# yaoyongxin/dmft-ed

Hardware: AMD Instinct MI355X
Metric: Lanczos SpMV GB/s + ground-state iters/s, Ns=16 half-filled sector, 1/2/4/8 GPU (higher is better)
Workload: dtype f64; 1 GPU; c2: Norb=1 Nbath=7 (Nlevels=16) half-filled (4,4) sector, dim 4900, stored real(8) H, plain Lanczos 512 iters/step, persistent MODE 4 (4 = stored matrix in the Kronecker register layout); parallelism=sector replicas x1

## Files before the change

dmft-ed_amd/csrc/ed_host.hpp:

```cpp
#pragma once
#include <hip/hip_runtime.h>
#include <stdint.h>

#include <string>

#include "../../include/ed_gpu.h"

std::string& ed_err_slot();
static inline int fail(int code, const std::string& msg) {
  ed_err_slot() = msg;
  return code;
}
#define HIPCK(x)                                                                       \
  do {                                                                                 \
    hipError_t e_ = (x);                                                               \
    if (e_ != hipSuccess)                                                              \
      return fail(ED_ERR_HIP, std::string(#x) + " -> " + hipGetErrorString(e_));       \
  } while (0)
#define CK(x)                  \
  do {                         \
    int r_ = (x);              \
    if (r_ != ED_OK) return r_; \
  } while (0)

namespace edg {

constexpr bool pkr_fits(int E, int RPT) { return RPT * (3 * E + 8) + 3 * E <= 216; }
constexpr bool pkr_fits_c512(int E, int RPT) { return E == 4 ? RPT <= 10 : RPT <= 6; }
constexpr int preg_cap(bool hc, bool vc) { return vc ? (hc ? 80 : 84) : 112; }
static inline int persist_rpt01(int64_t dim) {
  const int64_t rpt = (dim + 1024 - 1) / 1024;
  return rpt <= 6 ? (int)rpt : rpt <= 8 ? 8 : rpt <= 10 ? 10 : rpt <= 12 ? 12 : 16;
}

struct PersistGeom {
  int64_t dim = 0;
  int preg_E = 0, preg_rpt = 0, kreg_W = 0, kreg_rpt = 0, pkr_E = 0, pkr_rpt = 0;
};

int persist_launch(bool hc, bool vc, int mode, const PersistGeom& g, const void* run, int64_t lds,
                   hipStream_t st, int nb);

}
```

dmft-ed_amd/csrc/ed_lib.hip:

```cpp
#include <hip/hip_runtime.h>
#include <math.h>
#include <stdint.h>
#include <stdio.h>
#include <string.h>

#include <algorithm>
#include <atomic>
#include <condition_variable>
#include <functional>
#include <mutex>
#include <thread>
#include <string>
#include <map>
#include <vector>

#include "ed_kernels.hpp"
#include "ed_persist.hpp"
#include "ed_trlan.hpp"
#include "ed_trlbatch.hpp"
#include "ed_trlmulti.hpp"
#include "ed_fused.hpp"
#include "ed_split.hpp"
#include "ed_tables.hpp"
#include "ed_host.hpp"
// ... 92 lines not shown
  int split_uch = 8;
  SplitSlice* d_bsl = nullptr;
  int nbsl = 0;
  int2* d_itR = nullptr;
  int* d_glist = nullptr;
  int* d_xoff = nullptr;
  int2* d_ul = nullptr;
  uint32_t* d_lw = nullptr;
  int64_t nul = 0, nlw = 0, nfar = 0, nfar_u = 0;
  bool fused = false;
  FuUnit* d_fu = nullptr;
  int64_t nfu = 0;
  uint32_t* d_fa = nullptr;
  int2* d_ful = nullptr;
  uint32_t* d_flw = nullptr;
  int64_t fu_na = 0, fu_nu = 0, fu_nl = 0, fu_far = 0, fu_far_u = 0;
  int fu_wa_max = 0, fu_wa_min = 0, fu_uch = kFuUChunk;
  DirChunk* d_dchunk = nullptr;
  int ndchunk = 0;
  DirChunk* d_dchunk2 = nullptr;
  int ndchunk2 = 0;
  DirGroup* d_dops = nullptr;
  uint16_t *d_rank16 = nullptr, *d_pat16 = nullptr;
  void* d_ddiag = nullptr;
  bool dir_patlds = false;
  int dir_lds = 0, dir_grid = 0;
  bool kron = false;
  KronHost K;
  void *d_x = nullptr, *d_y = nullptr;
  LancWS ws;
  int64_t bytes = 0;
  std::vector<void*> allocs;
  double pthresh = 0.0;
  int preg_E = 0;
  int preg_rpt = 0;
  int kreg_W = 0, kreg_rpt = 0;
  uint32_t* d_pk = nullptr;
  void* d_dict = nullptr;
  int ndict = 0;
  int pkr_state = 0;
  int pkr_src = -1;
  int pkr_E = 0, pkr_rpt = 0, pkr_du = 0, pkr_dd = 0, pkr_degu = 0, pkr_degd = 0;
  const int32_t *d_kupc = nullptr, *d_kdwc = nullptr;
  const double *d_kupv = nullptr, *d_kdwv = nullptr, *d_kdiag = nullptr;
  hipGraphExec_t gexec = nullptr;
  int g_path = -2, g_vc = -1, g_chunk = 0;
  bool g_basis = false;
};

static int dcopy(const ed_sector* s, void* dst, const void* src, size_t n, hipMemcpyKind k) {
  HIPCK(hipMemcpyAsync(dst, src, n, k, s->stream));
  HIPCK(hipStreamSynchronize(s->stream));
  return ED_OK;
}
static int dalloc(ed_sector* s, void** p, size_t n) {
  if (n == 0) n = 16;
  hipError_t e = hipMallocAsync(p, n, s->stream);
  if (e != hipSuccess) {
    *p = nullptr;
    return fail(e == hipErrorOutOfMemory ? ED_ERR_OOM : ED_ERR_HIP,
                std::string("hipMalloc(") + std::to_string(n) + ") -> " + hipGetErrorString(e));
  }
  s->allocs.push_back(*p);
  s->bytes += (int64_t)n;
  return ED_OK;
}
static void dfree(ed_sector* s, void** p, size_t n) {
  if (!*p) return;
  auto it = std::find(s->allocs.begin(), s->allocs.end(), *p);
  if (it != s->allocs.end()) s->allocs.erase(it);
  (void)hipFreeAsync(*p, s->stream);
  s->bytes -= (int64_t)n;
  *p = nullptr;
}
template <class T>
static int dalloc_t(ed_sector* s, T** p, size_t count) {
  return dalloc(s, (void**)p, count * sizeof(T));
}
template <class T>
static int upload(ed_sector* s, T** p, const std::vector<T>& h) {
  CK(dalloc_t(s, p, h.size()));
  return dcopy(s, *p, h.data(), h.size() * sizeof(T), hipMemcpyHostToDevice);
}

static std::mutex g_pin_mu;
static std::multimap<size_t, void*> g_pin_free;
static std::map<void*, size_t> g_pin_size;
static void* pinned_get(size_t n) {
  {
    std::lock_guard<std::mutex> lk(g_pin_mu);
    auto it = g_pin_free.lower_bound(n);
    if (it != g_pin_free.end()) {
      void* p = it->second;
      g_pin_free.erase(it);
      return p;
    }
  }
  n = std::max<size_t>(n, 4096);
  void* p = nullptr;
  if (hipHostMalloc(&p, n, hipHostMallocDefault) != hipSuccess) return nullptr;
  std::lock_guard<std::mutex> lk(g_pin_mu);
  g_pin_size[p] = n;
  return p;
}
static void pinned_put(void* p) {
  if (!p) return;
  std::lock_guard<std::mutex> lk(g_pin_mu);
  g_pin_free.emplace(g_pin_size[p], p);
}
struct PinnedLease {
  void* const p;
  const hipStream_t st;
  PinnedLease(size_t n, hipStream_t st_) : p(pinned_get(n)), st(st_) {}
  PinnedLease(const PinnedLease&) = delete;
  ~PinnedLease() {
    if (!p) return;
    (void)hipStreamSynchronize(st);
    pinned_put(p);
  }
};
struct DevFree {
  void* p;
  hipStream_t st;
  ~DevFree() { (void)hipFreeAsync(p, st); }
};
static inline size_t even(size_t q) { return (q + 1) & ~(size_t)1; }

static void sector_free(ed_sector* s) {
  if (!s) return;
  (void)hipSetDevice(s->device);
  if (s->gexec) (void)hipGraphExecDestroy(s->gexec);
  for (hipEvent_t& e : s->ws.ev)
    if (e) (void)hipEventDestroy(e);
// ... 1578 lines not shown
  const int64_t du = K.dimup;
  std::vector<int32_t> uc((size_t)K.degup * du);
  std::vector<double> uv((size_t)K.degup * du);
  if (K.degup) {
    CK(dcopy(s, uc.data(), K.upc, uc.size() * 4, hipMemcpyDeviceToHost));
    CK(dcopy(s, uv.data(), K.upv, uv.size() * 8, hipMemcpyDeviceToHost));
  }
  std::vector<std::vector<PkrHop>> ul(du);
  for (int64_t r = 0; r < du; r++)
    for (int e = 0; e < K.degup; e++) {
      uint64_t bits;
      memcpy(&bits, &uv[(size_t)e * du + r], 8);
      ul[r].push_back({uc[(size_t)e * du + r], bits});
    }
  pkr_order_up(ul, (int)du, s->pkr_E);
  s->pkr_degu = s->pkr_E;
  CK(pkr_upload(s, ul, s->pkr_degu, du, &s->d_kupc, &s->d_kupv));
  s->d_kdwc = K.dwc;
  s->d_kdwv = (const double*)K.dwv;
  s->d_kdiag = nullptr;
  s->pkr_state = 1;
  return 1;
}

static int64_t persist_lds(const ed_sector* s, int vc, int mode);
static int64_t persist_vrows(const ed_sector* s, int mode, int vc = 0) {
  switch (mode) {
    case 2: return (int64_t)kPRegBlock * s->preg_rpt;
    case 3: return (int64_t)kPRegBlock * s->kreg_rpt;
    case 4: return (int64_t)kPRegBlock * s->pkr_rpt;
    default: return (int64_t)kPBlock * persist_rpt01(s->dim);
  }
}
static int persist_mode(ed_sector* s, int vc, int path) {
  const int o = s->opts;
  if (o & ED_OPT_NO_PERSIST) return -1;
  const int64_t vs = vc ? 16 : 8;
  const int64_t rpt_max = (vc || s->hc) ? 5 : 8;
  if (s->dim > rpt_max * (int64_t)kPBlock) return -1;
  int64_t lds = ((persist_vrows(s, 0) * vs + 15) & ~(int64_t)15);
  if (!(o & (ED_OPT_NO_PKRON | ED_OPT_NO_PREG)) &&
      ((path == 0 && !(o & ED_OPT_PERSIST_STORED) && build_pkron_stored(s) > 0) ||
       (path == 2 && build_pkron_direct(s) > 0)) &&
      (vc == 0 || pkr_fits_c512(s->pkr_E, s->pkr_rpt)) &&
      persist_lds(s, vc, 4) <= kLdsBudget)
    return 4;
  if (path == 0) {
    if (o & ED_OPT_PERSIST_STORED) return lds <= kLdsBudget ? 0 : -1;
    if (o & ED_OPT_NO_PREG) return -1;
    if (s->dim > 10 * (int64_t)kPRegBlock) return -1;
    const int W = build_preg(s);
    if (W < 0) return -1;
    if (s->preg_rpt * W > preg_cap(s->hc, vc)) return -1;
    if (persist_lds(s, vc, 2) > kLdsBudget) return -1;
    return 2;
  }
  if (path == 2 && !(o & ED_OPT_NO_PREG) && s->dim <= 10 * (int64_t)kPRegBlock) {
    const KronHost& K = s->K;
    const int deg = K.degup + K.degdw;
    int W = 0;
    for (int w : {8, 12, 14, 16})
      if (!W && deg <= w) W = w;
    const int64_t rpt = (s->dim + kPRegBlock - 1) / kPRegBlock;
    const int RPT = rpt <= 2 ? 2 : rpt <= 4 ? 4 : rpt <= 6 ? 6 : rpt <= 8 ? 8 : 10;
    const int64_t hs = s->hc ? 16 : 8;
    const int64_t dict = ((int64_t)(K.degup * K.dimup + K.degdw * K.dimdw) + 1) * hs;
    const int cap = preg_cap(s->hc, vc);
// ... 12 lines not shown
           (int64_t)K.nimp * K.nimp * 8 + 256;
    return lds <= kLdsBudget ? 1 : -1;
  }
  return -1;
}

static int64_t persist_lds(const ed_sector* s, int vc, int mode) {
  const int64_t vs = vc ? 16 : 8, vr = persist_vrows(s, mode, vc);
  int64_t lds = ((vr * vs + 15) & ~(int64_t)15);
  if (mode == 4) {
    if (!vc) return (((vr + vr / kPRegBlock) * vs + 15) & ~(int64_t)15);
    return lds + (int64_t)s->pkr_E * s->pkr_dd * 8;
  }
  if (mode == 2) {
    const int64_t hs = s->hc ? 16 : 8;
    return lds + ((vr * 8 + 15) & ~(int64_t)15) + (((int64_t)s->ndict * hs + 15) & ~(int64_t)15);
  }
  if (mode == 3) {
    const int64_t hs = s->hc ? 16 : 8;
    const int64_t dict = ((int64_t)(s->K.degup * s->K.dimup + s->K.degdw * s->K.dimdw) + 1) * hs;
    return lds + ((vr * 8 + 15) & ~(int64_t)15) + ((dict + 15) & ~(int64_t)15);
  }
  if (mode == 1) {
    const KronHost& K = s->K;
    const int64_t hs = s->hc ? 16 : 8;
    auto al = [](int64_t b) { return (b + 15) & ~(int64_t)15; };
    lds += al(K.dimup * hs) + al(K.dimdw * hs) + al((int64_t)K.degup * K.dimup * hs) +
           al((int64_t)K.degdw * K.dimdw * hs) + al((int64_t)K.degup * K.dimup * 4) +
           al((int64_t)K.degdw * K.dimdw * 4) + al(K.dimup) + al(K.dimdw) + al((int64_t)K.nimp * K.nimp * 8);
  }
  return lds;
}

static PersistGeom persist_geom(const ed_sector* s) {
  PersistGeom g;
  g.dim = s->dim;
  g.preg_E = s->preg_E;
  g.preg_rpt = s->preg_rpt;
  g.kreg_W = s->kreg_W;
  g.kreg_rpt = s->kreg_rpt;
  g.pkr_E = s->pkr_E;
  g.pkr_rpt = s->pkr_rpt;
  return g;
}

struct PersistBatch {
  int nb;
  void *R, *P;
  LancState* st;
  double *alpha, *beta;
  int64_t ldr, ldp, ldab;
};

template <bool VC>
static int persist_iters(ed_sector* s, int mode, bool basis, int niter, int first, hipStream_t st,
                         const PersistBatch* bt = nullptr) {
  LancWS& w = s->ws;
  const int nb = bt ? bt->nb : 1;
  auto fill = [&](auto& r) {
    using RT = std::remove_reference_t<decltype(r)>;
    using HT = std::remove_const_t<std::remove_pointer_t<decltype(r.diag)>>;
    memset(&r, 0, sizeof(RT));
    r.diag = (const HT*)s->d_diag;
    r.sptr = s->d_sptr;
    r.cols = s->d_cols;
    r.vals = (const HT*)s->d_vals;
    r.dim = s->dim;
    r.R = w.R;
    r.P = w.P;
    r.st = w.st;
    r.alpha = w.alpha;
    r.beta = w.beta;
    r.basis = basis ? w.basis : nullptr;
    r.niter = niter;
    r.first = first;
    r.thresh = s->pthresh;
    r.pk = s->d_pk;
    r.dict = (const HT*)s->d_dict;
    r.ndict = s->ndict;
    r.kupc = s->d_kupc;
    r.kupv = s->d_kupv;
    r.kdwc = s->d_kdwc;
    r.kdwv = s->d_kdwv;
    r.kdiag = s->d_kdiag;
    r.kdu = s->pkr_du;
    r.kdd = s->pkr_dd;
    r.kdegu = s->pkr_degu;
    r.kdegd = s->pkr_degd;
    if (bt) {
      r.R = bt->R;
      r.P = bt->P;
      r.st = bt->st;
      r.alpha = bt->alpha;
      r.beta = bt->beta;
      r.basis = nullptr;
      r.ldr = bt->ldr;
      r.ldp = bt->ldp;
      r.ldab = bt->ldab;
    }
  };
  const int64_t lds = persist_lds(s, VC, mode);
  if (s->hc) {
    if constexpr (!VC) return fail(ED_ERR_ARG, "complex H needs complex vectors");
    else {
      PersistRun<true> r;
      fill(r);
      if (mode == 1 || mode == 3) r.K = kron_args<true>(s);
      if (mode == 4) return fail(ED_ERR_UNSUPPORTED, "MODE 4 needs real H");
      return persist_launch(true, true, mode, persist_geom(s), &r, lds, st, nb);
    }
  }
  PersistRun<false> r;
  fill(r);
  if (mode == 1 || mode == 3 || (mode == 4 && s->kron)) r.K = kron_args<false>(s);
  return persist_launch(false, VC, mode, persist_geom(s), &r, lds, st, nb);
}

static int persist_set_thresh(ed_sector* s, double thresh, hipStream_t st) {
  s->pthresh = thresh;
  HIPCK(hipMemsetAsync(s->ws.st, 0, sizeof(LancState), st));
  HIPCK(hipMemsetAsync(s->ws.alpha, 0, 2 * (s->ws.cap + 2) * sizeof(double), st));
  return ED_OK;
}


__global__ void k_hash_vec(double* v, int64_t n, uint64_t seed) {
  for (int64_t i = (int64_t)blockIdx.x * kBlock + threadIdx.x; i < n; i += (int64_t)gridDim.x * kBlock) {
    v[i] = hash_vec_unit(i, seed);
  }
}

template <bool VC>
struct Trlan {
  using V = val_t<VC>;
  ed_sector* s = nullptr;
  int path = 0;
  hipStream_t st = nullptr;
  int64_t dim = 0;
  int G = 1, m = 0, mcap = 0;
  bool fused = true;
  V *Vb = nullptr, *Xb = nullptr, *w = nullptr;
  double2 *h = nullptr, *coef = nullptr, *part = nullptr, *part2 = nullptr;
  int kFinFoldG = 256;
  bool graphs_on = true;
  bool solo = true;
  bool locupd = true;
  int* lof = nullptr;
  double *Y = nullptr, *npart = nullptr, *alpha = nullptr, *beta = nullptr;
  double *npA = nullptr, *npB = nullptr;
  double* hp = nullptr;
  std::vector<void*> mine;
  std::vector<std::pair<int, hipGraphExec_t>> graphs;
  int nhv = 0;
  ~Trlan() {
// ... 1040 lines not shown
  if (hipStreamSynchronize(s->stream) != hipSuccess) {
    sector_free(s);
    return fail(ED_ERR_HIP, "sector build");
  }
#undef TRY
  *out = s;
  return ED_OK;
}

int ed_sector_create(const ed_params* p, int32_t q1, int32_t q2, int32_t flags, int32_t device,
                     void* stream, ed_sector** out) {
  return sector_create(p, q1, q2, flags, 0, -1, device, (hipStream_t)stream, out);
}

int ed_sector_create_rows(const ed_params* p, int32_t q1, int32_t q2, int32_t flags, int64_t row0,
                          int64_t nrows, int32_t device, void* stream, ed_sector** out) {
  return sector_create(p, q1, q2, flags, row0, nrows, device, (hipStream_t)stream, out);
}

int ed_sector_destroy(ed_sector* s) {
  sector_free(s);
  return ED_OK;
}

static constexpr int32_t kOptKnown =
    ED_OPT_NO_PERSIST | ED_OPT_PERSIST_STORED | ED_OPT_NO_PREG | ED_OPT_NO_PKRON | ED_OPT_SPLIT_SIMPLE |
    ED_OPT_NO_BATCH | ED_OPT_EIGH_NO_VERIFY | ED_OPT_TRLAN_UNFUSED | ED_OPT_TRLAN_NOFOLD | ED_OPT_NO_GRAPH |
    ED_OPT_TRLAN_NOLOCAL | ED_OPT_TRLAN_NOSOLO | ED_OPT_TRLAN_FULLUPD | ED_OPT_STORED_EXACT |
    ED_OPT_EIGH_FULLPROBE | ED_OPT_NO_FUSED | ED_OPT_EIGH_NOHINT;

int ed_sector_set_options(ed_sector* s, int32_t opts) {
  if (!s) return fail(ED_ERR_ARG, "null");
  if (opts & ~kOptKnown) return fail(ED_ERR_ARG, "unknown ED_OPT_* bits");
  if (opts != s->opts) drop_graph(s);
  s->opts = opts;
  return ED_OK;
}

int ed_sector_get_info(const ed_sector* s, ed_sector_info* info) {
  if (!s || !info) return fail(ED_ERR_ARG, "null");
  memset(info, 0, sizeof(*info));
  info->dim = s->dim;
  info->row0 = s->row0;
  info->nrows = s->nrows;
  info->nnz = (s->flags & ED_STORED) ? s->nnz : 0;
  info->padded = s->padded;
  info->ns = s->Mh.ns;
  info->mode = s->Mh.mode;
  info->q1 = s->T.q1;
  info->q2 = s->T.q2;
  info->flags = s->flags;
  info->kron = s->kron ? 1 : 0;
  info->dimup = s->T.dimup;
  info->dimdw = s->T.dimdw;
  info->device_bytes = s->bytes;
  info->packed = s->d_words ? 1 : 0;
  info->npdict = s->npdict;
  info->split = s->split ? 1 : 0;
  info->split_far = s->nfar;
  info->split_far_uniform = s->nfar_u;
  info->fused = s->fused ? 1 : 0;
  info->fused_far = s->fu_far;
  info->fused_far_uniform = s->fu_far_u;
  info->fused_bytes = s->fused ? (s->fu_na + s->fu_nl) * 4 + s->fu_nu * 8 + s->nfu * (int64_t)sizeof(FuUnit) : 0;
  info->split_bytes = s->split ? (s->paddedA + s->nlw) * 4 + s->nul * 8 + s->split_meta : 0;
  info->split_list_bytes = s->split ? s->split_listR : 0;
  return ED_OK;
// ... 92 lines not shown
    cols[q] = (int32_t)(s->row0 + i);
    vals[2 * q] = dg[hw * i];
    vals[2 * q + 1] = hw == 2 ? dg[2 * i + 1] : 0.0;
    q++;
    int64_t base = sptr[i >> 6] + (i & 63);
    for (int k = 0; k < cnt[i]; k++) {
      int64_t t = base + 64 * (int64_t)k;
      cols[q] = sc[t];
      vals[2 * q] = sv[hw * t];
      vals[2 * q + 1] = hw == 2 ? sv[2 * t + 1] : 0.0;
      q++;
    }
    rowptr[i + 1] = q;
  }
  return ED_OK;
}

int ed_sector_sell_view(const ed_sector* s, ed_sell_view* v) {
  if (!s || !v) return fail(ED_ERR_ARG, "null");
  if (!(s->flags & ED_STORED)) return fail(ED_ERR_STATE, "sector was built without ED_STORED");
  v->dim = s->dim;
  v->nslice = s->nslice;
  v->slots = s->padded;
  v->value_bytes = s->hc ? 16 : 8;
  v->pad = 0;
  v->diag = s->d_diag;
  v->sptr = s->d_sptr;
  v->cols = s->d_cols;
  v->vals = s->d_vals;
  v->rowcnt = s->d_cnt;
  return ED_OK;
}

struct LancDriver {
  ed_sector* s;
  int vc, path, pm;
  bool basis;
  hipStream_t st;
  int start(double thresh) {
    if (pm >= 0) return persist_set_thresh(s, thresh, st);
    return vc ? lanc_start<true>(s, thresh, st) : lanc_start<false>(s, thresh, st);
  }
  int iters(int n, bool first) {
    if (pm >= 0)
      return vc ? persist_iters<true>(s, pm, basis, n, first ? 1 : 0, st)
                : persist_iters<false>(s, pm, basis, n, first ? 1 : 0, st);
    return vc ? lanc_iters<true>(s, path, basis, n, st) : lanc_iters<false>(s, path, basis, n, st);
  }
};

static int make_driver(ed_sector* s, int vtype, bool basis, LancDriver* d) {
  CK(whole_only(s));
  d->s = s;
  d->vc = vtype ? 1 : 0;
  if (d->vc == 0 && s->hc) return fail(ED_ERR_ARG, "complex H needs vtype=1");
  d->path = resolve_path(s, -1);
  d->pm = persist_mode(s, d->vc, d->path);
  d->basis = basis;
  d->st = s->stream;
  return ED_OK;
}

static int lanc_load_start(ed_sector* s, int vc, const void* v0, bool v0_device) {
  const size_t vs = vc ? 16 : 8;
  if (v0) {
    HIPCK(hipMemcpyAsync(s->ws.R, v0, s->dim * vs,
                         v0_device ? hipMemcpyDeviceToDevice : hipMemcpyHostToDevice, s->stream));
  } else {
    hipLaunchKernelGGL(k_default_start, dim3(grid_for(s->dim * (vc ? 2 : 1))), dim3(kBlock), 0,
                       s->stream, (double*)s->ws.R, s->dim * (vc ? 2 : 1));
    HIPCK(hipGetLastError());
  }
  return ED_OK;
}

int ed_sector_lanc_run(ed_sector* s, int32_t vtype, const void* v0_dev, int32_t niter,
                       double* alfa, double* beta, float* ms, void* stream) {
  (void)stream;
  if (!s || niter < 1) return fail(ED_ERR_ARG, "bad args");
  HIPCK(hipSetDevice(s->device));
  LancDriver d;
  CK(make_driver(s, vtype, false, &d));
  CK(lanc_prepare(s, d.vc, niter, false, 0));
  CK(lanc_load_start(s, d.vc, v0_dev, true));
  LancWS& w = s->ws;
  for (hipEvent_t& e : w.ev)
    if (!e) HIPCK(hipEventCreate(&e));
  hipEvent_t e0 = w.ev[0], e1 = w.ev[1];
  int rc = d.start(1e-300);
  if (rc == ED_OK) {
    HIPCK(hipEventRecord(e0, d.st));
    rc = d.iters(niter, true);
    HIPCK(hipEventRecord(e1, d.st));
  }
  const size_t nab = (size_t)w.cap + 2 + niter;
  if (rc == ED_OK && (alfa || beta))
    HIPCK(hipMemcpyAsync(w.h_ab, w.alpha, nab * sizeof(double), hipMemcpyDeviceToHost, d.st));
  HIPCK(hipStreamSynchronize(d.st));
  CK(rc);
  if (alfa) memcpy(alfa, w.h_ab, niter * sizeof(double));
  if (beta) memcpy(beta, w.h_ab + w.cap + 2, niter * sizeof(double));
  if (ms) HIPCK(hipEventElapsedTime(ms, e0, e1));
  return ED_OK;
}

int ed_sector_lanc_tridiag(ed_sector* s, int32_t vtype, const void* v0, int32_t nitermax,
                           double threshold, double* alfa, double* beta, int32_t* nlanc) {
  if (!s || !alfa || !beta || nitermax < 1) return fail(ED_ERR_ARG, "bad args");
  HIPCK(hipSetDevice(s->device));
  LancDriver d;
  CK(make_driver(s, vtype, false, &d));
  CK(lanc_prepare(s, d.vc, nitermax, false, 0));
  CK(lanc_load_start(s, d.vc, v0, false));
  CK(d.start(threshold));
  CK(d.iters(nitermax, true));
  std::vector<double> a(nitermax + 1), b(nitermax + 2);
  HIPCK(hipMemcpyAsync(a.data(), s->ws.alpha, nitermax * 8, hipMemcpyDeviceToHost, d.st));
  HIPCK(hipMemcpyAsync(b.data(), s->ws.beta, (nitermax + 1) * 8, hipMemcpyDeviceToHost, d.st));
  LancState hs;
  HIPCK(hipMemcpyAsync(&hs, s->ws.st, sizeof(hs), hipMemcpyDeviceToHost, d.st));
  HIPCK(hipStreamSynchronize(d.st));
  int n = hs.iter;
  for (int q = 0; q < nitermax; q++) {
    alfa[q] = q < n ? a[q] : 0.0;
    beta[q] = (q >= 1 && q <= n) ? b[q] : 0.0;
  }
  beta[0] = 0.0;
  if (nlanc) *nlanc = n;
  return ED_OK;
}

int ed_sector_lanc_tridiag_batch(ed_sector* s, int32_t vtype, int32_t nseed, const void* v0_dev,
                                 int32_t nitermax, double threshold, double* alfa, double* beta,
                                 int32_t* nlanc) {
  if (!s || !v0_dev || !alfa || !beta || nitermax < 1 || nseed < 1) return fail(ED_ERR_ARG, "bad args");
  HIPCK(hipSetDevice(s->device));
  LancDriver d;
  CK(make_driver(s, vtype, false, &d));
  const size_t vs = d.vc ? 16 : 8;
  auto unpack = [&](int k, const double* a, const double* b, int n) {
    double* al = alfa + (size_t)k * nitermax;
    double* be = beta + (size_t)k * nitermax;
    for (int q = 0; q < nitermax; q++) {
      al[q] = q < n ? a[q] : 0.0;
      be[q] = (q >= 1 && q <= n) ? b[q] : 0.0;
    }
    be[0] = 0.0;
    if (nlanc) nlanc[k] = n;
  };
  if (d.pm < 0 || (s->opts & ED_OPT_NO_BATCH)) {
    CK(lanc_prepare(s, d.vc, nitermax, false, 0));
    for (int k = 0; k < nseed; k++) {
      CK(lanc_load_start(s, d.vc, (const unsigned char*)v0_dev + (size_t)k * s->dim * vs, true));
      CK(d.start(threshold));
      CK(d.iters(nitermax, true));
      std::vector<double> a(nitermax + 1), b(nitermax + 2);
      LancState hs;
      HIPCK(hipMemcpyAsync(a.data(), s->ws.alpha, nitermax * 8, hipMemcpyDeviceToHost, d.st));
      HIPCK(hipMemcpyAsync(b.data(), s->ws.beta, (nitermax + 1) * 8, hipMemcpyDeviceToHost, d.st));
      HIPCK(hipMemcpyAsync(&hs, s->ws.st, sizeof(hs), hipMemcpyDeviceToHost, d.st));
      HIPCK(hipStreamSynchronize(d.st));
      unpack(k, a.data(), b.data(), hs.iter);
    }
    return ED_OK;
  }
  CK(lanc_prepare(s, d.vc, nitermax, false, 0));
  PersistBatch bt;
  bt.nb = nseed;
  bt.ldr = s->dim;
  bt.ldp = (int64_t)p_rows(s);
  bt.ldab = 2 * ((int64_t)nitermax + 2);
  hipStream_t st = d.st;
  void *R = nullptr, *P = nullptr, *ab = nullptr, *sts = nullptr;
  HIPCK(hipMallocAsync(&R, (size_t)nseed * bt.ldr * vs, st));
  HIPCK(hipMallocAsync(&P, (size_t)nseed * bt.ldp * vs, st));
  HIPCK(hipMallocAsync(&ab, (size_t)nseed * bt.ldab * 8, st));
  HIPCK(hipMallocAsync(&sts, (size_t)nseed * sizeof(LancState), st));
  auto release = [&]() {
    (void)hipFreeAsync(R, st);
    (void)hipFreeAsync(P, st);
    (void)hipFreeAsync(ab, st);
    (void)hipFreeAsync(sts, st);
  };
  bt.R = R;
  bt.P = P;
  bt.st = (LancState*)sts;
  bt.alpha = (double*)ab;
  bt.beta = (double*)ab + nitermax + 2;
  s->pthresh = threshold;
  int rc = ED_OK;
  if (hipMemcpyAsync(R, v0_dev, (size_t)nseed * s->dim * vs, hipMemcpyDeviceToDevice, st) != hipSuccess ||
      hipMemsetAsync(P, 0, (size_t)nseed * bt.ldp * vs, st) != hipSuccess ||
      hipMemsetAsync(ab, 0, (size_t)nseed * bt.ldab * 8, st) != hipSuccess ||
      hipMemsetAsync(sts, 0, (size_t)nseed * sizeof(LancState), st) != hipSuccess)
    rc = fail(ED_ERR_HIP, "batch workspace");
  if (rc == ED_OK)
    rc = d.vc ? persist_iters<true>(s, d.pm, false, nitermax, 1, st, &bt)
              : persist_iters<false>(s, d.pm, false, nitermax, 1, st, &bt);
  std::vector<double> hab((size_t)nseed * bt.ldab);
  std::vector<LancState> hst(nseed);
  if (rc == ED_OK) {
    HIPCK(hipMemcpyAsync(hab.data(), ab, hab.size() * 8, hipMemcpyDeviceToHost, st));
    HIPCK(hipMemcpyAsync(hst.data(), sts, nseed * sizeof(LancState), hipMemcpyDeviceToHost, st));
  }
  release();
  HIPCK(hipStreamSynchronize(st));
  CK(rc);
  for (int k = 0; k < nseed; k++) {
    const double* a = hab.data() + (size_t)k * bt.ldab;
    unpack(k, a, a + nitermax + 2, hst[k].iter);
  }
  return ED_OK;
}

static int check_op_target(const ed_sector* src, const ed_sector* dst, int32_t op, int32_t level) {
  if (!src || !dst) return fail(ED_ERR_ARG, "null");
  if (src->device != dst->device) return fail(ED_ERR_ARG, "sectors on different devices");
  if (op != 0 && op != 1) return fail(ED_ERR_ARG, "op must be 0 (c) or 1 (c^+)");
  if (level < 0 || level >= 2 * src->Mh.ns || src->Mh.ns != dst->Mh.ns)
    return fail(ED_ERR_ARG, "level outside the 2*Ns Fock levels / mismatched models");
  const int ns = src->Mh.ns, d = op == 1 ? 1 : -1, up = level < ns;
  int e1 = src->T.q1, e2 = src->T.q2;
  if (src->Mh.mode == ED_MODE_NORMAL) {
    if (up) e1 += d; else e2 += d;
  } else if (src->Mh.mode == ED_MODE_SUPERC) {
    e1 += up ? d : -d;
  } else {
    e1 += d;
    if (src->Mh.jz) e2 += d * (src->Mh.lz2[up ? level : level - ns] + (up ? 1 : -1));
  }
  if (dst->Mh.mode != src->Mh.mode || dst->Mh.jz != src->Mh.jz || dst->T.q1 != e1 || dst->T.q2 != e2)
// ... 159 lines not shown
    fr[f].pad = 0.0;
    np += npole[f];
  }
  const size_t bf = fr.size() * sizeof(GfFrac), be = (size_t)std::max<int64_t>(np, 1) * 8;
  std::vector<unsigned char> hb(bf + 2 * be);
  memcpy(hb.data(), fr.data(), bf);
  if (np) {
    memcpy(hb.data() + bf, E, np * 8);
    memcpy(hb.data() + bf + be, z, np * 8);
  }
  hipStream_t st = (hipStream_t)stream;
  void* d = nullptr;
  HIPCK(hipMallocAsync(&d, hb.size(), st));
  HIPCK(hipMemcpyAsync(d, hb.data(), hb.size(), hipMemcpyHostToDevice, st));
  const unsigned char* db = (const unsigned char*)d;
  const int nt = lmats + lreal;
  hipLaunchKernelGGL(k_gf_poles, dim3((nt + kBlock - 1) / kBlock), dim3(kBlock), 0, st, (const GfFrac*)db, nfrac,
                     (const double*)(db + bf), (const double*)(db + bf + be), wm, lmats, wr, lreal, eps,
                     (double2*)gm, (double2*)gr);
  const hipError_t le = hipGetLastError();
  (void)hipFreeAsync(d, st);
  HIPCK(hipStreamSynchronize(st));
  HIPCK(le);
  return ED_OK;
}

int ed_sector_lanc_tridiag_dev(ed_sector* s, int32_t vtype, const void* v0_dev, int32_t nitermax,
                               double threshold, double* alfa, double* beta, int32_t* nlanc) {
  if (!s || !alfa || !beta || !v0_dev || nitermax < 1) return fail(ED_ERR_ARG, "bad args");
  HIPCK(hipSetDevice(s->device));
  LancDriver d;
  CK(make_driver(s, vtype, false, &d));
  CK(lanc_prepare(s, d.vc, nitermax, false, 0));
  CK(lanc_load_start(s, d.vc, v0_dev, true));
  CK(d.start(threshold));
  CK(d.iters(nitermax, true));
  std::vector<double> a(nitermax + 1), b(nitermax + 2);
  HIPCK(hipMemcpyAsync(a.data(), s->ws.alpha, nitermax * 8, hipMemcpyDeviceToHost, d.st));
  HIPCK(hipMemcpyAsync(b.data(), s->ws.beta, (nitermax + 1) * 8, hipMemcpyDeviceToHost, d.st));
  LancState hs;
  HIPCK(hipMemcpyAsync(&hs, s->ws.st, sizeof(hs), hipMemcpyDeviceToHost, d.st));
  HIPCK(hipStreamSynchronize(d.st));
  int n = hs.iter;
  for (int q = 0; q < nitermax; q++) {
    alfa[q] = q < n ? a[q] : 0.0;
    beta[q] = (q >= 1 && q <= n) ? b[q] : 0.0;
  }
  beta[0] = 0.0;
  if (nlanc) *nlanc = n;
  return ED_OK;
}

int ed_sector_lanc_eigh(ed_sector* s, int32_t vtype, const void* v0, int32_t nitermax,
                        double threshold, int32_t ncheck, double* egs, void* vect,
                        int32_t* nlanc) {
  if (!s || !egs || nitermax < 1) return fail(ED_ERR_ARG, "bad args");
  if (ncheck < 1) ncheck = 10;
  HIPCK(hipSetDevice(s->device));
  const int vc = vtype ? 1 : 0;
  const size_t vs = vc ? 16 : 8;
  size_t fr = 0, tot = 0;
  HIPCK(hipMemGetInfo(&fr, &tot));
  const bool keep = vect && ((double)nitermax * s->dim * vs < 0.25 * (double)fr);
  LancDriver d;
  CK(make_driver(s, vtype, keep, &d));
  CK(lanc_prepare(s, vc, nitermax, keep, keep ? nitermax : 0));
  CK(lanc_load_start(s, vc, v0, false));
  CK(d.start(threshold));
  std::vector<double> a(nitermax + 2, 0.0), b(nitermax + 2, 0.0), esave;
  int done_iters = 0, nl = 0;
  bool stop = false;
  const int chunk = d.pm >= 0 ? 64 : 32;
  while (!stop && done_iters < nitermax) {
    int n = std::min(chunk, nitermax - done_iters);
    const int expected = done_iters + n;
    CK(d.iters(n, done_iters == 0));
    HIPCK(hipMemcpyAsync(a.data(), s->ws.alpha, nitermax * 8, hipMemcpyDeviceToHost, d.st));
    HIPCK(hipMemcpyAsync(b.data(), s->ws.beta, (nitermax + 1) * 8, hipMemcpyDeviceToHost, d.st));
    LancState hs;
    HIPCK(hipMemcpyAsync(&hs, s->ws.st, sizeof(hs), hipMemcpyDeviceToHost, d.st));
    HIPCK(hipStreamSynchronize(d.st));
    int have = hs.iter;
    for (int it = done_iters + 1; it <= have && !stop; it++) {
      if (fabs(b[it]) < threshold) { stop = true; break; }
      nl = it;
      if (nl >= ncheck) {
        double e0 = lowest_ritz(a, b, nl);
        esave.push_back(e0);
        if (esave.size() >= 2 && fabs(esave.back() - esave[esave.size() - 2]) <= threshold) stop = true;
      }
    }
    if (hs.done) stop = true;
    if (have < expected && !hs.done) return fail(ED_ERR_STATE, "Lanczos iteration count mismatch");
    done_iters = have;
  }
  if (nl == 0) {
    LancState hs;
    CK(dcopy(s, &hs, s->ws.st, sizeof(hs), hipMemcpyDeviceToHost));
    char msg[256];
    snprintf(msg, sizeof msg,
             "Lanczos made no step: iter=%d done=%d beta0=%g b[1]=%g a[0]=%g path=%d pm=%d keep=%d",
             hs.iter, hs.done, hs.beta, b[1], a[0], d.path, d.pm, (int)keep);
    return fail(ED_ERR_STATE, msg);
  }
  std::vector<double> dg(a.begin(), a.begin() + nl), e(nl, 0.0), z((size_t)nl * nl, 0.0);
  for (int q = 1; q < nl; q++) e[q] = b[q];
  for (int q = 0; q < nl; q++) z[q + (size_t)nl * q] = 1.0;
  if (nl > 0) tql2(nl, dg.data(), e.data(), z.data());
  *egs = nl > 0 ? dg[0] : 0.0;
  if (nlanc) *nlanc = nl;
  if (vect && nl > 0) {
    LancWS& w = s->ws;
    HIPCK(hipMemcpyAsync(w.z, z.data(), nl * 8, hipMemcpyHostToDevice, s->stream));
    RedSlot slot{w.partials, w.counter + 2};
// ... 259 lines not shown
```

dmft-ed_amd/csrc/ed_persist.hpp:

```cpp
#pragma once
#include "ed_kernels.hpp"

namespace edg {

constexpr int kPBlock = 1024;
constexpr int kPChunk = 8;
constexpr int kPRegBlock = 512;

template <bool HC>
struct PersistRun {
  using H = val_t<HC>;
  const H* diag;
  const int64_t* sptr;
  const int32_t* cols;
  const H* vals;
  KronArgs<HC> K;
  int64_t dim;
  void* R;
  void* P;
  LancState* st;
  double* alpha;
  double* beta;
  void* basis;
  const uint32_t* pk;
  const H* dict;
  int ndict;
  const int32_t* kupc;
  const double* kupv;
  const int32_t* kdwc;
  const double* kdwv;
  const double* kdiag;
  int kdu, kdd, kdegu, kdegd;
  double thresh;
  int niter;
  int first;
  int64_t ldr, ldp;
  int64_t ldab;
};

template <int CTRL, int RM>
__device__ __forceinline__ double dpp_add(double v) {
  const int lo = __double2loint(v), hi = __double2hiint(v);
  const int l2 = __builtin_amdgcn_mov_dpp(lo, CTRL, RM, 0xF, true);
  const int h2 = __builtin_amdgcn_mov_dpp(hi, CTRL, RM, 0xF, true);
  return v + __hiloint2double(h2, l2);
}
__device__ __forceinline__ double wave_sum_dpp(double v) {
  v = dpp_add<0xB1, 0xF>(v);
  v = dpp_add<0x4E, 0xF>(v);
  v = dpp_add<0x141, 0xF>(v);
  v = dpp_add<0x140, 0xF>(v);
// ... 29 lines not shown
  } else {
    return *(const __attribute__((address_space(3))) T*)(uintptr_t)a;
  }
}

struct PRows {
  int row0, stride, nvalid, iu;
};

template <int MODE, int RPT, int NT>
__device__ __forceinline__ PRows persist_rows(int tid, int64_t dim, int du, int dd) {
  PRows q;
  if constexpr (MODE == 4) {
    const int G = NT / du;
    if (tid < G * du) {
      const int g = tid / du;
      q.iu = tid - g * du;
      q.row0 = g * du + q.iu;
      q.stride = G * du;
      q.nvalid = dd > g ? (dd - g + G - 1) / G : 0;
    } else {
      q.iu = 0;
      q.row0 = G * du * RPT + (tid - G * du);
      q.stride = NT - G * du;
      q.nvalid = 0;
    }
  } else {
    q.iu = 0;
    q.row0 = tid;
    q.stride = NT;
    q.nvalid = dim > tid ? (int)((dim - tid + NT - 1) / NT) : 0;
  }
  return q;
}

template <bool HC, bool VC, int MODE, int RPT, int E = 1, int NT = kPBlock>
__global__ void __launch_bounds__(NT) k_lanc_persist(const PersistRun<HC> a) {
  using V = val_t<VC>;
  using H = val_t<HC>;
  extern __shared__ __align__(16) unsigned char smem[];
  __shared__ double ws[NT / 64];
  __shared__ double ws2[NT / 64];
  constexpr int VROWS = NT * RPT;
  constexpr bool SLOT = MODE == 4 && !VC;
  constexpr int VSLOT = NT + 1;
  constexpr int VLDS = SLOT ? RPT * VSLOT : VROWS;
  V* vl = (V*)smem;
  const int64_t dim = a.dim;
  const int tid = threadIdx.x;
  const int run = blockIdx.x;
  V* Rg = (V*)a.R + run * a.ldr;
  V* Pg = (V*)a.P + run * a.ldp;
  LancState* st = a.st + run;
  PRows q = persist_rows<MODE, RPT, NT>(tid, dim, a.kdu, a.kdd);
#define PROW(r) (q.row0 + (r) * q.stride)
#define LPOS(r) (SLOT ? (r) * VSLOT + tid : PROW(r))

  const H* aup = nullptr;
  const H* adw = nullptr;
  const H* upv = nullptr;
  const H* dwv = nullptr;
  const int32_t* upc = nullptr;
  const int32_t* dwc = nullptr;
  const uint8_t* impu = nullptr;
  const uint8_t* impd = nullptr;
  const double* uimp = nullptr;
// ... 127 lines not shown
        int pos;
        if (ok) {
          const int iw2 = a.kdwc[e * dd + iw], r2 = iw2 / G;
          pos = SLOT ? r2 * VSLOT + (iw2 - r2 * G) * du + q.iu : iw2 * du + q.iu;
        } else {
          pos = okr ? 0 : LPOS(r);
        }
        dcol[r * E + e] = (SLOT ? lb : 0u) + (uint32_t)pos * (uint32_t)sizeof(V);
        if constexpr (!(KR && VC)) dval[r * E + e] = ok ? a.kdwv[e * dd + iw] : 0.0;
      }
      {
        double d = 0.0;
        if (okr) {
          if (a.kdiag) {
            d = a.kdiag[PROW(r)];
          } else {
            const KronArgs<HC>& K = a.K;
            d = re_of(add(add(K.aup[q.iu], K.adw[iw]), mk<HC>(K.uimp[K.impu[q.iu] * K.nimp + K.impd[iw]], 0.0)));
          }
        }
        dgr[r] = d;
      }
    }
  }

  constexpr bool PG = (REG || KRC) && VC;
  constexpr bool PIPE = KR && !VC && RPT * E <= 40;
  constexpr bool UREG = !VC && (REG || (KR && (!PIPE || RPT * E < 40)));
  V u[UREG ? RPT : 1];
  V p[PG ? 1 : RPT];
  uint32_t rix[RPT];
  double b, s;
  int it0;
  {
    double nrm = 0.0;
#pragma unroll
    for (int r = 0; r < RPT; r++) {
      const int i = PROW(r);
      const bool ok = r < q.nvalid;
      const V x = ok ? Rg[i] : vzero<V>();
      if constexpr (UREG) u[r] = x;
      vl[LPOS(r)] = x;
      if constexpr (!PG) p[r] = (ok && !a.first) ? Pg[i] : vzero<V>();
      if (a.first) {
        nrm += redot(x, x);
        if constexpr (PG) Pg[i] = vzero<V>();
      }
      if constexpr (MODE == 1) {
        const uint32_t w_ = (uint32_t)(i / a.K.dimup);
        rix[r] = ok ? (w_ << 16) | (uint32_t)(i - (int64_t)w_ * a.K.dimup) : 0u;
      }
    }
    if (a.first) {
      const double n2 = pblock_sum<NT>(nrm, ws);
      if (n2 == 0.0) {
        if (tid == 0) { st->iter = 0; st->done = 1; st->beta = 0.0; }
        return;
      }
      s = 1.0 / sqrt(n2);
      b = 0.0;
      it0 = 0;
      if (tid == 0) {
        st->iter = 0;
        st->done = 0;
        st->beta = 0.0;
      }
    } else {
      b = st->beta;
      s = 1.0 / b;
      it0 = st->iter;
    }
    __syncthreads();
  }
  if (st->done && !a.first) return;
  const double thresh = a.thresh;
  double* const alpha_out = a.alpha + run * a.ldab;
  double* const beta_out = a.beta + run * a.ldab;
  V* const basis = run == 0 ? (V*)a.basis : nullptr;

  double gu[PIPE ? E : 1], gd[PIPE ? E : 1], go = 0.0;
  auto gather = [&](int r, double* hu, double* hd, double& ho) {
    if constexpr (PIPE) {
#pragma unroll
      for (int e = 0; e < E; e++) hu[e] = lds_ldv<double>(ucol[e] + r * VSLOT * 8);
#pragma unroll
      for (int e = 0; e < E; e++) hd[e] = lds_ldv<double>(dcol[r * E + e]);
      if constexpr (UREG) ho = u[r];
      else ho = vl[LPOS(r)];
    }
  };
  gather(0, gu, gd, go);

  for (int k = 0; k < a.niter; k++) {
    const int it = it0 + k;
    if constexpr (REG) {
#pragma unroll
      for (int e = 0; e < RPT * E; e++) asm volatile("" : "+v"(pk[e]));
    }
    if constexpr (KR) {
#pragma unroll
      for (int e = 0; e < RPT * E; e++) asm volatile("" : "+v"(dcol[e]));
    }
    asm volatile("" : "+v"(q.row0));
    V w[RPT];
    double ap = 0.0;
    if constexpr (PIPE) {
#pragma unroll
      for (int r = 0; r < RPT; r++) {
        double nu[E], nd[E], no = 0.0;
        if (r + 1 < RPT) gather(r + 1, nu, nd, no);
// ... 133 lines not shown
      } else if constexpr (!PIPE) {
        p[r] = x;
      }
      if constexpr (UREG) u[r] = w[r];
      vl[LPOS(r)] = w[r];
    }
#ifdef ED_P4_NOBETA
    __syncthreads();
    const double bsq = 1.0 + bp * 1e-300;
#else
    const double bsq = pblock_sum<NT, false>(bp, ws2);
#endif
    if constexpr (PIPE) {
      gather(0, gu, gd, go);
      __builtin_amdgcn_sched_barrier(0);
    }
#ifdef ED_P4_NOBETA
    const double bn = bsq;
#else
    const double bn = sqrt(bsq);
#endif
    if (tid == 0) {
      alpha_out[it] = alpha;
      beta_out[it + 1] = bn;
    }
    b = bn;
    s = 1.0 / bn;
    if (bn < thresh) {
      if (tid == 0) {
        st->done = 1;
        st->iter = it + 1;
        st->beta = bn;
      }
      return;
    }
  }
#pragma unroll
  for (int r = 0; r < RPT; r++) {
    if (r < q.nvalid) {
      Rg[PROW(r)] = UREG ? u[r] : vl[LPOS(r)];
      if constexpr (!PG) Pg[PROW(r)] = p[r];
    }
  }
  if (tid == 0) {
    st->iter = it0 + a.niter;
    st->beta = b;
  }
#undef PROW
#undef LPOS
}

}
```

dmft-ed_amd/csrc/ed_persist_launch.hip:

```cpp
#include "ed_host.hpp"
#include "ed_kernels.hpp"
#include "ed_persist.hpp"

namespace edg {

template <bool HC, bool VC, int MODE, int RPT, int E = 1>
static int persist_launch_t(const PersistGeom& s, const PersistRun<HC>& run, int64_t lds, hipStream_t st, int nb) {
  if constexpr ((MODE == 2 || MODE == 3) && RPT * E > preg_cap(HC, VC)) {
    return fail(ED_ERR_UNSUPPORTED, "register-resident ELL exceeds the spill-free budget");
  } else if constexpr (MODE == 4 && (HC || (VC ? !pkr_fits_c512(E, RPT) : !pkr_fits(E, RPT)))) {
    return fail(ED_ERR_UNSUPPORTED, "Kronecker register layout: real H within the register budget");
  } else {
  constexpr int NT = MODE >= 2 ? kPRegBlock : kPBlock;
  auto fn = k_lanc_persist<HC, VC, MODE, RPT, E, NT>;
  HIPCK(hipFuncSetAttribute((const void*)fn, hipFuncAttributeMaxDynamicSharedMemorySize, (int)lds));
  hipLaunchKernelGGL(fn, dim3(nb), dim3(NT), (size_t)lds, st, run);
  HIPCK(hipGetLastError());
  return ED_OK;
  }
}

template <bool HC, bool VC, int MODE, int W>
static int persist_launch_e(const PersistGeom& s, const PersistRun<HC>& run, int64_t lds, hipStream_t st, int nb) {
  switch (MODE == 2 ? s.preg_rpt : MODE == 3 ? s.kreg_rpt : s.pkr_rpt) {
    case 2: return persist_launch_t<HC, VC, MODE, 2, W>(s, run, lds, st, nb);
    case 4: return persist_launch_t<HC, VC, MODE, 4, W>(s, run, lds, st, nb);
    case 6: return persist_launch_t<HC, VC, MODE, 6, W>(s, run, lds, st, nb);
    case 8: return persist_launch_t<HC, VC, MODE, 8, W>(s, run, lds, st, nb);
    default: return persist_launch_t<HC, VC, MODE, 10, W>(s, run, lds, st, nb);
  }
}

template <bool HC, bool VC, int MODE>
static int persist_launch_m(const PersistGeom& s, const PersistRun<HC>& run, int64_t lds, hipStream_t st, int nb = 1) {
  if constexpr (MODE == 4) {
    if constexpr (HC) {
      return fail(ED_ERR_UNSUPPORTED, "MODE 4 needs a real H");
    } else {
      return s.pkr_E == 4 ? persist_launch_e<HC, VC, 4, 4>(s, run, lds, st, nb)
                           : persist_launch_e<HC, VC, 4, 8>(s, run, lds, st, nb);
    }
  } else if constexpr (MODE >= 2) {
    switch (MODE == 2 ? s.preg_E : s.kreg_W) {
      case 8: return persist_launch_e<HC, VC, MODE, 8>(s, run, lds, st, nb);
      case 12: return persist_launch_e<HC, VC, MODE, 12>(s, run, lds, st, nb);
      case 14: return persist_launch_e<HC, VC, MODE, 14>(s, run, lds, st, nb);
      default: return persist_launch_e<HC, VC, MODE, 16>(s, run, lds, st, nb);
    }
// ... 41 lines not shown
```

Measured before the change: 581,700 Lanczos iters/s.

## Cut per-call host overhead in persistent Lanczos launch and result fetch

Caches the persistent-mode choice and its LDS size per sector, and calls hipFuncSetAttribute only when the required LDS grows on a device. The persistent kernel now writes alpha/beta straight into mapped pinned host memory, reads the start vector in place from the caller's device pointer, and zeroes its own tail, so several memsets and memcpys per call go away. The aim is fewer HIP API calls and copies around short Lanczos runs. The costs are host-mapped writes from the kernel over the interconnect and the risk of a stale cached attribute or mode.

```diff
diff --git a/dmft-ed_amd/csrc/ed_host.hpp b/dmft-ed_amd/csrc/ed_host.hpp
--- a/dmft-ed_amd/csrc/ed_host.hpp
+++ b/dmft-ed_amd/csrc/ed_host.hpp
@@ -36,6 +36,7 @@
 struct PersistGeom {
   int64_t dim = 0;
   int preg_E = 0, preg_rpt = 0, kreg_W = 0, kreg_rpt = 0, pkr_E = 0, pkr_rpt = 0;
+  int device = 0;
 };
 
 int persist_launch(bool hc, bool vc, int mode, const PersistGeom& g, const void* run, int64_t lds,
diff --git a/dmft-ed_amd/csrc/ed_lib.hip b/dmft-ed_amd/csrc/ed_lib.hip
--- a/dmft-ed_amd/csrc/ed_lib.hip
+++ b/dmft-ed_amd/csrc/ed_lib.hip
@@ -148,6 +148,10 @@
   int64_t bytes = 0;
   std::vector<void*> allocs;
   double pthresh = 0.0;
+  struct {
+    int vc = -1, path = -3, opts = 0, mode = -1;
+    int64_t lds = 0;
+  } pchoice;
   int preg_E = 0;
   int preg_rpt = 0;
   int kreg_W = 0, kreg_rpt = 0;
@@ -214,7 +218,7 @@
   }
   n = std::max<size_t>(n, 4096);
   void* p = nullptr;
-  if (hipHostMalloc(&p, n, hipHostMallocDefault) != hipSuccess) return nullptr;
+  if (hipHostMalloc(&p, n, hipHostMallocPortable | hipHostMallocMapped) != hipSuccess) return nullptr;
   std::lock_guard<std::mutex> lk(g_pin_mu);
   g_pin_size[p] = n;
   return p;
@@ -1859,7 +1863,7 @@
     default: return (int64_t)kPBlock * persist_rpt01(s->dim);
   }
 }
-static int persist_mode(ed_sector* s, int vc, int path) {
+static int persist_mode_derive(ed_sector* s, int vc, int path) {
   const int o = s->opts;
   if (o & ED_OPT_NO_PERSIST) return -1;
   const int64_t vs = vc ? 16 : 8;
@@ -1938,6 +1942,19 @@
   return lds;
 }
 
+static int persist_mode(ed_sector* s, int vc, int path) {
+  auto& c = s->pchoice;
+  if (c.vc == vc && c.path == path && c.opts == s->opts) return c.mode;
+  c.vc = -1;
+  const int mode = persist_mode_derive(s, vc, path);
+  c.lds = mode >= 0 ? persist_lds(s, vc, mode) : 0;
+  c.mode = mode;
+  c.path = path;
+  c.opts = s->opts;
+  c.vc = vc;
+  return mode;
+}
+
 static PersistGeom persist_geom(const ed_sector* s) {
   PersistGeom g;
   g.dim = s->dim;
@@ -1947,6 +1964,7 @@
   g.kreg_rpt = s->kreg_rpt;
   g.pkr_E = s->pkr_E;
   g.pkr_rpt = s->pkr_rpt;
+  g.device = s->device;
   return g;
 }
 
@@ -1960,7 +1978,7 @@
 
 template <bool VC>
 static int persist_iters(ed_sector* s, int mode, bool basis, int niter, int first, hipStream_t st,
-                         const PersistBatch* bt = nullptr) {
+                         const PersistBatch* bt = nullptr, const void* v0 = nullptr, bool host_ab = false) {
   LancWS& w = s->ws;
   const int nb = bt ? bt->nb : 1;
   auto fill = [&](auto& r) {
@@ -1973,10 +1991,11 @@
     r.vals = (const HT*)s->d_vals;
     r.dim = s->dim;
     r.R = w.R;
+    r.v0 = first ? v0 : nullptr;
     r.P = w.P;
     r.st = w.st;
-    r.alpha = w.alpha;
-    r.beta = w.beta;
+    r.alpha = host_ab ? w.h_ab : w.alpha;
+    r.beta = host_ab ? w.h_ab + w.cap + 2 : w.beta;
     r.basis = basis ? w.basis : nullptr;
     r.niter = niter;
     r.first = first;
@@ -2005,7 +2024,8 @@
       r.ldab = bt->ldab;
     }
   };
-  const int64_t lds = persist_lds(s, VC, mode);
+  const auto& pc = s->pchoice;
+  const int64_t lds = (pc.vc == (int)VC && pc.mode == mode) ? pc.lds : persist_lds(s, VC, mode);
   if (s->hc) {
     if constexpr (!VC) return fail(ED_ERR_ARG, "complex H needs complex vectors");
     else {
@@ -2023,9 +2043,8 @@
 }
 
 static int persist_set_thresh(ed_sector* s, double thresh, hipStream_t st) {
+  (void)st;
   s->pthresh = thresh;
-  HIPCK(hipMemsetAsync(s->ws.st, 0, sizeof(LancState), st));
-  HIPCK(hipMemsetAsync(s->ws.alpha, 0, 2 * (s->ws.cap + 2) * sizeof(double), st));
   return ED_OK;
 }
 
@@ -3132,7 +3151,10 @@
 int ed_sector_set_options(ed_sector* s, int32_t opts) {
   if (!s) return fail(ED_ERR_ARG, "null");
   if (opts & ~kOptKnown) return fail(ED_ERR_ARG, "unknown ED_OPT_* bits");
-  if (opts != s->opts) drop_graph(s);
+  if (opts != s->opts) {
+    drop_graph(s);
+    s->pchoice.vc = -1;
+  }
   s->opts = opts;
   return ED_OK;
 }
@@ -3291,6 +3313,8 @@
   return ED_OK;
 }
 
+static int lanc_load_start(ed_sector* s, int vc, const void* v0, bool v0_device);
+
 struct LancDriver {
   ed_sector* s;
   int vc, path, pm;
@@ -3300,11 +3324,33 @@
     if (pm >= 0) return persist_set_thresh(s, thresh, st);
     return vc ? lanc_start<true>(s, thresh, st) : lanc_start<false>(s, thresh, st);
   }
-  int iters(int n, bool first) {
+  int iters(int n, bool first, const void* v0 = nullptr) {
     if (pm >= 0)
-      return vc ? persist_iters<true>(s, pm, basis, n, first ? 1 : 0, st)
-                : persist_iters<false>(s, pm, basis, n, first ? 1 : 0, st);
+      return vc ? persist_iters<true>(s, pm, basis, n, first ? 1 : 0, st, nullptr, v0, true)
+                : persist_iters<false>(s, pm, basis, n, first ? 1 : 0, st, nullptr, v0, true);
     return vc ? lanc_iters<true>(s, path, basis, n, st) : lanc_iters<false>(s, path, basis, n, st);
+  }
+  int fetch(double* a, int na, double* b, int nb, LancState* hs) {
+    LancWS& w = s->ws;
+    if (pm < 0) {
+      HIPCK(hipMemcpyAsync(a, w.alpha, (size_t)na * 8, hipMemcpyDeviceToHost, st));
+      HIPCK(hipMemcpyAsync(b, w.beta, (size_t)nb * 8, hipMemcpyDeviceToHost, st));
+    }
+    HIPCK(hipMemcpyAsync(hs, w.st, sizeof(*hs), hipMemcpyDeviceToHost, st));
+    HIPCK(hipStreamSynchronize(st));
+    if (pm >= 0) {
+      memcpy(a, w.h_ab, (size_t)na * 8);
+      memcpy(b, w.h_ab + w.cap + 2, (size_t)nb * 8);
+    }
+    return ED_OK;
+  }
+  int load(const void* v0, bool v0_device, const void** inplace) {
+    *inplace = nullptr;
+    if (pm >= 0 && v0 && v0_device) {
+      *inplace = v0;
+      return ED_OK;
+    }
+    return lanc_load_start(s, vc, v0, v0_device);
   }
 };
 
@@ -3341,7 +3387,8 @@
   LancDriver d;
   CK(make_driver(s, vtype, false, &d));
   CK(lanc_prepare(s, d.vc, niter, false, 0));
-  CK(lanc_load_start(s, d.vc, v0_dev, true));
+  const void* v0p = nullptr;
+  CK(d.load(v0_dev, true, &v0p));
   LancWS& w = s->ws;
   for (hipEvent_t& e : w.ev)
     if (!e) HIPCK(hipEventCreate(&e));
@@ -3349,11 +3396,11 @@
   int rc = d.start(1e-300);
   if (rc == ED_OK) {
     HIPCK(hipEventRecord(e0, d.st));
-    rc = d.iters(niter, true);
+    rc = d.iters(niter, true, v0p);
     HIPCK(hipEventRecord(e1, d.st));
   }
   const size_t nab = (size_t)w.cap + 2 + niter;
-  if (rc == ED_OK && (alfa || beta))
+  if (rc == ED_OK && (alfa || beta) && d.pm < 0)
     HIPCK(hipMemcpyAsync(w.h_ab, w.alpha, nab * sizeof(double), hipMemcpyDeviceToHost, d.st));
   HIPCK(hipStreamSynchronize(d.st));
   CK(rc);
@@ -3374,11 +3421,8 @@
   CK(d.start(threshold));
   CK(d.iters(nitermax, true));
   std::vector<double> a(nitermax + 1), b(nitermax + 2);
-  HIPCK(hipMemcpyAsync(a.data(), s->ws.alpha, nitermax * 8, hipMemcpyDeviceToHost, d.st));
-  HIPCK(hipMemcpyAsync(b.data(), s->ws.beta, (nitermax + 1) * 8, hipMemcpyDeviceToHost, d.st));
   LancState hs;
-  HIPCK(hipMemcpyAsync(&hs, s->ws.st, sizeof(hs), hipMemcpyDeviceToHost, d.st));
-  HIPCK(hipStreamSynchronize(d.st));
+  CK(d.fetch(a.data(), nitermax, b.data(), nitermax + 1, &hs));
   int n = hs.iter;
   for (int q = 0; q < nitermax; q++) {
     alfa[q] = q < n ? a[q] : 0.0;
@@ -3410,15 +3454,13 @@
   if (d.pm < 0 || (s->opts & ED_OPT_NO_BATCH)) {
     CK(lanc_prepare(s, d.vc, nitermax, false, 0));
     for (int k = 0; k < nseed; k++) {
-      CK(lanc_load_start(s, d.vc, (const unsigned char*)v0_dev + (size_t)k * s->dim * vs, true));
+      const void* v0p = nullptr;
+      CK(d.load((const unsigned char*)v0_dev + (size_t)k * s->dim * vs, true, &v0p));
       CK(d.start(threshold));
-      CK(d.iters(nitermax, true));
+      CK(d.iters(nitermax, true, v0p));
       std::vector<double> a(nitermax + 1), b(nitermax + 2);
       LancState hs;
-      HIPCK(hipMemcpyAsync(a.data(), s->ws.alpha, nitermax * 8, hipMemcpyDeviceToHost, d.st));
-      HIPCK(hipMemcpyAsync(b.data(), s->ws.beta, (nitermax + 1) * 8, hipMemcpyDeviceToHost, d.st));
-      HIPCK(hipMemcpyAsync(&hs, s->ws.st, sizeof(hs), hipMemcpyDeviceToHost, d.st));
-      HIPCK(hipStreamSynchronize(d.st));
+      CK(d.fetch(a.data(), nitermax, b.data(), nitermax + 1, &hs));
       unpack(k, a.data(), b.data(), hs.iter);
     }
     return ED_OK;
@@ -3447,15 +3489,8 @@
   bt.alpha = (double*)ab;
   bt.beta = (double*)ab + nitermax + 2;
   s->pthresh = threshold;
-  int rc = ED_OK;
-  if (hipMemcpyAsync(R, v0_dev, (size_t)nseed * s->dim * vs, hipMemcpyDeviceToDevice, st) != hipSuccess ||
-      hipMemsetAsync(P, 0, (size_t)nseed * bt.ldp * vs, st) != hipSuccess ||
-      hipMemsetAsync(ab, 0, (size_t)nseed * bt.ldab * 8, st) != hipSuccess ||
-      hipMemsetAsync(sts, 0, (size_t)nseed * sizeof(LancState), st) != hipSuccess)
-    rc = fail(ED_ERR_HIP, "batch workspace");
-  if (rc == ED_OK)
-    rc = d.vc ? persist_iters<true>(s, d.pm, false, nitermax, 1, st, &bt)
-              : persist_iters<false>(s, d.pm, false, nitermax, 1, st, &bt);
+  int rc = d.vc ? persist_iters<true>(s, d.pm, false, nitermax, 1, st, &bt, v0_dev)
+                : persist_iters<false>(s, d.pm, false, nitermax, 1, st, &bt, v0_dev);
   std::vector<double> hab((size_t)nseed * bt.ldab);
   std::vector<LancState> hst(nseed);
   if (rc == ED_OK) {
@@ -3681,15 +3716,13 @@
   LancDriver d;
   CK(make_driver(s, vtype, false, &d));
   CK(lanc_prepare(s, d.vc, nitermax, false, 0));
-  CK(lanc_load_start(s, d.vc, v0_dev, true));
+  const void* v0p = nullptr;
+  CK(d.load(v0_dev, true, &v0p));
   CK(d.start(threshold));
-  CK(d.iters(nitermax, true));
+  CK(d.iters(nitermax, true, v0p));
   std::vector<double> a(nitermax + 1), b(nitermax + 2);
-  HIPCK(hipMemcpyAsync(a.data(), s->ws.alpha, nitermax * 8, hipMemcpyDeviceToHost, d.st));
-  HIPCK(hipMemcpyAsync(b.data(), s->ws.beta, (nitermax + 1) * 8, hipMemcpyDeviceToHost, d.st));
   LancState hs;
-  HIPCK(hipMemcpyAsync(&hs, s->ws.st, sizeof(hs), hipMemcpyDeviceToHost, d.st));
-  HIPCK(hipStreamSynchronize(d.st));
+  CK(d.fetch(a.data(), nitermax, b.data(), nitermax + 1, &hs));
   int n = hs.iter;
   for (int q = 0; q < nitermax; q++) {
     alfa[q] = q < n ? a[q] : 0.0;
@@ -3724,11 +3757,8 @@
     int n = std::min(chunk, nitermax - done_iters);
     const int expected = done_iters + n;
     CK(d.iters(n, done_iters == 0));
-    HIPCK(hipMemcpyAsync(a.data(), s->ws.alpha, nitermax * 8, hipMemcpyDeviceToHost, d.st));
-    HIPCK(hipMemcpyAsync(b.data(), s->ws.beta, (nitermax + 1) * 8, hipMemcpyDeviceToHost, d.st));
     LancState hs;
-    HIPCK(hipMemcpyAsync(&hs, s->ws.st, sizeof(hs), hipMemcpyDeviceToHost, d.st));
-    HIPCK(hipStreamSynchronize(d.st));
+    CK(d.fetch(a.data(), nitermax, b.data(), nitermax + 1, &hs));
     int have = hs.iter;
     for (int it = done_iters + 1; it <= have && !stop; it++) {
       if (fabs(b[it]) < threshold) { stop = true; break; }
diff --git a/dmft-ed_amd/csrc/ed_persist.hpp b/dmft-ed_amd/csrc/ed_persist.hpp
--- a/dmft-ed_amd/csrc/ed_persist.hpp
+++ b/dmft-ed_amd/csrc/ed_persist.hpp
@@ -17,6 +17,7 @@
   KronArgs<HC> K;
   int64_t dim;
   void* R;
+  const void* v0;
   void* P;
   LancState* st;
   double* alpha;
@@ -112,6 +113,14 @@
     q.nvalid = dim > tid ? (int)((dim - tid + NT - 1) / NT) : 0;
   }
   return q;
+}
+
+template <int NT>
+__device__ __forceinline__ void persist_clear_tail(double* alpha, double* beta, int from, int end) {
+  for (int j = from + (int)threadIdx.x; j < end; j += NT) {
+    alpha[j] = 0.0;
+    beta[j + 1] = 0.0;
+  }
 }
 
 template <bool HC, bool VC, int MODE, int RPT, int E = 1, int NT = kPBlock>
@@ -305,13 +314,16 @@
   uint32_t rix[RPT];
   double b, s;
   int it0;
+  double* const alpha_out = a.alpha + run * a.ldab;
+  double* const beta_out = a.beta + run * a.ldab;
   {
+    const V* const Sg = (a.first && a.v0) ? (const V*)a.v0 + run * a.ldr : Rg;
     double nrm = 0.0;
 #pragma unroll
     for (int r = 0; r < RPT; r++) {
       const int i = PROW(r);
       const bool ok = r < q.nvalid;
-      const V x = ok ? Rg[i] : vzero<V>();
+      const V x = ok ? Sg[i] : vzero<V>();
       if constexpr (UREG) u[r] = x;
       vl[LPOS(r)] = x;
       if constexpr (!PG) p[r] = (ok && !a.first) ? Pg[i] : vzero<V>();
@@ -327,7 +339,8 @@
     if (a.first) {
       const double n2 = pblock_sum<NT>(nrm, ws);
       if (n2 == 0.0) {
-        if (tid == 0) { st->iter = 0; st->done = 1; st->beta = 0.0; }
+        if (tid == 0) { st->iter = 0; st->done = 1; st->beta = 0.0; beta_out[0] = 0.0; }
+        persist_clear_tail<NT>(alpha_out, beta_out, 0, a.niter);
         return;
       }
       s = 1.0 / sqrt(n2);
@@ -337,6 +350,7 @@
         st->iter = 0;
         st->done = 0;
         st->beta = 0.0;
+        beta_out[0] = 0.0;
       }
     } else {
       b = st->beta;
@@ -347,8 +361,6 @@
   }
   if (st->done && !a.first) return;
   const double thresh = a.thresh;
-  double* const alpha_out = a.alpha + run * a.ldab;
-  double* const beta_out = a.beta + run * a.ldab;
   V* const basis = run == 0 ? (V*)a.basis : nullptr;
 
   double gu[PIPE ? E : 1], gd[PIPE ? E : 1], go = 0.0;
@@ -548,6 +560,7 @@
         st->iter = it + 1;
         st->beta = bn;
       }
+      persist_clear_tail<NT>(alpha_out, beta_out, it + 1, it0 + a.niter);
       return;
     }
   }
diff --git a/dmft-ed_amd/csrc/ed_persist_launch.hip b/dmft-ed_amd/csrc/ed_persist_launch.hip
--- a/dmft-ed_amd/csrc/ed_persist_launch.hip
+++ b/dmft-ed_amd/csrc/ed_persist_launch.hip
@@ -1,8 +1,13 @@
+#include <atomic>
+#include <mutex>
+
 #include "ed_host.hpp"
 #include "ed_kernels.hpp"
 #include "ed_persist.hpp"
 
 namespace edg {
+
+constexpr int kMaxDevices = 64;
 
 template <bool HC, bool VC, int MODE, int RPT, int E = 1>
 static int persist_launch_t(const PersistGeom& s, const PersistRun<HC>& run, int64_t lds, hipStream_t st, int nb) {
@@ -13,7 +18,18 @@
   } else {
   constexpr int NT = MODE >= 2 ? kPRegBlock : kPBlock;
   auto fn = k_lanc_persist<HC, VC, MODE, RPT, E, NT>;
-  HIPCK(hipFuncSetAttribute((const void*)fn, hipFuncAttributeMaxDynamicSharedMemorySize, (int)lds));
+  static std::atomic<int64_t> lds_set[kMaxDevices];
+  static std::mutex mu;
+  const int dev = s.device;
+  if (dev < 0 || dev >= kMaxDevices) {
+    HIPCK(hipFuncSetAttribute((const void*)fn, hipFuncAttributeMaxDynamicSharedMemorySize, (int)lds));
+  } else if (lds > lds_set[dev].load(std::memory_order_acquire)) {
+    std::lock_guard<std::mutex> lk(mu);
+    if (lds > lds_set[dev].load(std::memory_order_relaxed)) {
+      HIPCK(hipFuncSetAttribute((const void*)fn, hipFuncAttributeMaxDynamicSharedMemorySize, (int)lds));
+      lds_set[dev].store(lds, std::memory_order_release);
+    }
+  }
   hipLaunchKernelGGL(fn, dim3(nb), dim3(NT), (size_t)lds, st, run);
   HIPCK(hipGetLastError());
   return ED_OK;
```

After: 591,100 Lanczos iters/s (median of 6 runs). 1.6% higher.
